# Schaudge/cellranger

Measured on AMD Instinct MI355X. Metric: M reads/sec barcode-correct+UMI-count, higher is better.
Workload: dtype u32/u64 integer keys; f64 posterior

## Files before the change

### cellranger_amd/csrc/common.h

```cpp
#pragma once

#include <hip/hip_runtime.h>

#include <cstdarg>
#include <cstdint>
#include <cstdio>
#include <cstring>
#include <map>
#include <mutex>
#include <set>
#include <string>
#include <vector>

#include "../../include/crgpu.h"

#define CR_WAVE 64
#define CR_SCALAR_N_WITHOUT_FLAGS 40

struct WlTables {
    bool set = false;
    uint32_t n = 0;
    uint32_t bitsA = 0;
    uint32_t bitsB = 0;
    uint32_t *d_offA = nullptr;
// ... 227 lines not shown
        if (_rc != CRGPU_OK) return _rc; \
    } while (0)

#define CR_REQUIRE(ctx, cond, code, ...)                     \
    do {                                                     \
        if (!(cond)) return cr_fail((ctx), (code), __VA_ARGS__); \
    } while (0)

int cr_scratch(crgpu_ctx *ctx, uint64_t bytes, void **out);
void cr_invalidate_range(crgpu_ctx *ctx, const void *p, uint64_t bytes);
void cr_drop_miss_records(crgpu_ctx *ctx);
void cr_drop_miss_records(crgpu_ctx *ctx, MissRecords &r);
bool cr_sweep_plan(uint32_t lo_bit, uint32_t hi_bit, SweepPlan *plan, uint32_t *widths);
uint32_t cr_sort_low_bits(uint32_t total_bits, uint32_t umi_bits);
bool cr_sort_finish_experiment();
int cr_order_runs(crgpu_ctx *ctx, uint64_t *d_keys, uint32_t *d_vals, uint64_t n, uint32_t low_bits, bool *fell_back);
static inline void cr_allow_lds(crgpu_ctx *ctx, const void *kernel, size_t bytes) {
    size_t &have = ctx->lds_attr_done[kernel];
    if (bytes > have) {
        (void)hipFuncSetAttribute(kernel, hipFuncAttributeMaxDynamicSharedMemorySize, (int)bytes);
        have = bytes;
    }
}

int cr_pool_alloc(crgpu_ctx *ctx, void **out, uint64_t bytes);
void cr_pool_free(crgpu_ctx *ctx, void *p);
void cr_pool_release_all(crgpu_ctx *ctx);

hipEvent_t cr_take_event(crgpu_ctx *ctx);
struct CrTimer {
    crgpu_ctx *ctx;
// ... 31 lines not shown
```

### cellranger_amd/csrc/dedup.hip

```cpp
#include "block_utils.h"
#include "common.h"

int cr_scan_small(crgpu_ctx *ctx, uint32_t *d_data, uint64_t n, uint32_t *d_total_out);
int cr_partition_by_owner(crgpu_ctx *ctx, const uint64_t *d_in, uint64_t *d_out, uint64_t n, uint32_t sh_bc,
                          uint32_t n_ranks, const uint32_t *bounds, uint64_t *counts_out);

#define NONE32 0xFFFFFFFFu

struct crgpu_counts {
    uint64_t n_triplets = 0, n_molecules = 0;
    uint32_t *d_bc = nullptr, *d_feature = nullptr, *d_count = nullptr;
    uint64_t *d_mkeys = nullptr;
    uint32_t *d_mreads = nullptr;
    uint32_t *d_corr_reads = nullptr;
    uint32_t *d_filt_reads = nullptr;
    int32_t *d_mprobe = nullptr;
    uint32_t *d_back = nullptr;
    uint32_t n_back = 0;
    uint32_t n_canon = 0;
    KeyLayout layout;
};

extern "C" int crgpu_set_key_layout(crgpu_ctx *ctx, uint32_t n_features, uint32_t umi_len, uint32_t n_libs,
                                    uint32_t multiplexing_lib_mask) {
// ... 604 lines not shown
            const uint64_t i = base + (uint64_t)j * CP_BLOCK + threadIdx.x;
            c += (f[j] && i < hi) ? 1u : 0u;
        }
    }
#pragma unroll
    for (int d = 32; d >= 1; d >>= 1) c += __shfl_xor(c, d);
    if ((threadIdx.x & 63u) == 0) ws[threadIdx.x >> 6] = c;
    __syncthreads();
    if (threadIdx.x == 0) {
        uint32_t t = 0;
        for (int w = 0; w < CP_WAVES; w++) t += ws[w];
        block_counts[blockIdx.x] = t;
    }
}

template <typename Flag, typename Emit>
__global__ __launch_bounds__(CP_BLOCK) void k_cp_write(Flag flag, Emit emit, uint64_t n, uint64_t tile,
                                                       const uint32_t *__restrict__ block_offs) {
    __shared__ uint32_t ws[CP_ITEMS * CP_WAVES];
    __shared__ uint32_t round_total;
    const uint32_t lane = threadIdx.x & 63u, wave = threadIdx.x >> 6;
    const uint64_t lo = (uint64_t)blockIdx.x * tile;
    const uint64_t hi = lo + tile < n ? lo + tile : n;
    uint32_t run = block_offs[blockIdx.x];
    for (uint64_t base = lo; base < hi; base += CP_ROUND) {
        bool f[CP_ITEMS];
        typename Emit::Pre pre[CP_ITEMS];
#pragma unroll
        for (int j = 0; j < CP_ITEMS; j++) {
            const uint64_t i = base + (uint64_t)j * CP_BLOCK + threadIdx.x;
            f[j] = flag(i < hi ? i : hi - 1);
            pre[j] = emit.pre(i < hi ? i : hi - 1);
        }
        uint32_t below[CP_ITEMS];
#pragma unroll
        for (int j = 0; j < CP_ITEMS; j++) {
            const uint64_t i = base + (uint64_t)j * CP_BLOCK + threadIdx.x;
            f[j] = f[j] && i < hi;
            const unsigned long long m = __ballot(f[j]);
// ... 28 lines not shown
    if (nb < 1) nb = 1;
    if (nb > 4096) nb = 4096;
    uint64_t tile = (n + nb - 1) / nb;
    tile = (tile + CP_ROUND - 1) / CP_ROUND * CP_ROUND;
    nb = (n + tile - 1) / tile;
    if (nb < 1) nb = 1;
    *tile_out = tile;
    return (uint32_t)nb;
}

template <typename Flag, typename Emit>
static int compact(crgpu_ctx *ctx, Flag flag, Emit emit, uint64_t n, uint32_t *d_block, uint32_t *d_total_out) {
    uint64_t tile;
    const uint32_t nb = cp_blocks(n, &tile);
    hipLaunchKernelGGL(k_cp_count<Flag>, dim3(nb), dim3(CP_BLOCK), 0, ctx->stream, flag, n, tile, d_block);
    CR_TRY(cr_scan_small(ctx, d_block, nb, d_total_out));
    hipLaunchKernelGGL((k_cp_write<Flag, Emit>), dim3(nb), dim3(CP_BLOCK), 0, ctx->stream, flag, emit, n, tile, d_block);
    CR_HIP(ctx, hipGetLastError());
    return CRGPU_OK;
}

#define ST_CORRECTED 1u
#define ST_LOW 2u
__device__ __forceinline__ uint32_t st_inc1(uint32_t s) { return s >> 2; }
__device__ __forceinline__ void st_or(uint16_t *st, uint64_t k, uint32_t bits) {
    atomicOr(reinterpret_cast<uint32_t *>(st) + (k >> 1), bits << (16u * (uint32_t)(k & 1u)));
}
__device__ __forceinline__ void move_reads(uint32_t *corr, uint16_t *st, uint32_t *inc_all, uint32_t *minidx, uint64_t k,
                                           uint32_t target, uint32_t my_cnt) {
    corr[k] = target;
    st_or(st, k, ST_CORRECTED);
    atomicAdd(reinterpret_cast<uint32_t *>(st) + (target >> 1), 4u << (16u * (target & 1u)));
// ... 142 lines not shown
            c += (head && i < hi) ? 1u : 0u;
        }
    }
#pragma unroll
    for (int d = 32; d >= 1; d >>= 1) c += __shfl_xor(c, d);
    if (lane == 0) ws[wave] = c;
    __syncthreads();
    if (threadIdx.x == 0) {
        uint32_t t = 0;
        for (int w = 0; w < CP_WAVES; w++) t += ws[w];
        block_counts[blockIdx.x] = t;
    }
}

__global__ __launch_bounds__(CP_BLOCK) void k_rl_write(const uint64_t *__restrict__ keys, const uint32_t shift, const uint64_t n,
                                                       const uint64_t tile, const uint32_t *__restrict__ block_offs,
                                                       uint64_t *__restrict__ ukey, uint32_t *__restrict__ upos,
                                                       uint16_t *__restrict__ z_st, uint32_t *__restrict__ z_inc,
                                                       uint32_t *__restrict__ z_min) {
    __shared__ uint32_t ws[CP_ITEMS * CP_WAVES];
    __shared__ uint32_t round_total;
    const uint32_t lane = threadIdx.x & 63u, wave = threadIdx.x >> 6;
    const uint64_t lo = (uint64_t)blockIdx.x * tile;
    const uint64_t hi = lo + tile < n ? lo + tile : n;
    uint32_t run = block_offs[blockIdx.x];
    for (uint64_t base = lo; base < hi; base += CP_ROUND) {
        uint64_t key[CP_ITEMS];
        bool f[CP_ITEMS];
        uint32_t below[CP_ITEMS];
        const uint64_t w0 = base + (uint64_t)wave * (64u * CP_ITEMS);
        const uint64_t wb = w0 > 0 ? (w0 - 1 < n ? w0 - 1 : n - 1) : 0;
        uint64_t carry_key = keys[wb];
        bool carry_valid = w0 > 0;
#pragma unroll
        for (int j = 0; j < CP_ITEMS; j++) {
            const uint64_t i = w0 + (uint64_t)j * 64 + lane;
            key[j] = keys[i < hi ? i : hi - 1];
        }
#pragma unroll
        for (int j = 0; j < CP_ITEMS; j++) {
// ... 10 lines not shown
#pragma unroll
            for (int d = 1; d < CP_ITEMS * CP_WAVES; d <<= 1) {
                const uint32_t y = __shfl_up(x, d);
                if (threadIdx.x >= (uint32_t)d) x += y;
            }
            ws[threadIdx.x] = x - v;
            if (threadIdx.x == CP_ITEMS * CP_WAVES - 1) round_total = x;
        }
        __syncthreads();
#pragma unroll
        for (int j = 0; j < CP_ITEMS; j++)
            if (f[j]) {
                const uint32_t o = run + ws[wave * CP_ITEMS + j] + below[j];
                ukey[o] = key[j];
                upos[o] = (uint32_t)(w0 + (uint64_t)j * 64 + lane);
                if (z_st) {
                    z_st[o] = 0;
                    z_inc[o] = 0u;
                    z_min[o] = 0xFFFFFFFFu;
                }
            }
        run += round_total;
        __syncthreads();
    }
}

static int run_lengths(crgpu_ctx *ctx, const uint64_t *keys, uint32_t shift, uint64_t n, uint64_t *ukey, uint32_t *upos,
                       uint32_t *d_block, uint32_t *d_total_out, uint16_t *z_st = nullptr, uint32_t *z_inc = nullptr,
                       uint32_t *z_min = nullptr) {
    uint64_t tile;
    const uint32_t nb = cp_blocks(n, &tile);
    hipLaunchKernelGGL(k_rl_count, dim3(nb), dim3(CP_BLOCK), 0, ctx->stream, keys, shift, n, tile, d_block);
    CR_TRY(cr_scan_small(ctx, d_block, nb, d_total_out));
    hipLaunchKernelGGL(k_rl_write, dim3(nb), dim3(CP_BLOCK), 0, ctx->stream, keys, shift, n, tile, d_block, ukey, upos, z_st, z_inc,
                       z_min);
    CR_HIP(ctx, hipGetLastError());
    return CRGPU_OK;
}

struct MtCarry {
    uint64_t prefix;
    bool has_mol;
    bool valid;
};

template <typename Flag>
__device__ __forceinline__ MtCarry mt_carry_from_memory(const Flag &flag, const uint64_t *__restrict__ ukey, uint32_t sh_feat,
                                                        uint64_t nd, uint64_t i0) {
    MtCarry c{0ull, false, false};
    if (i0 == 0 || i0 >= nd) return c;
// ... 783 lines not shown
        ~Guard() {
            if (armed) crgpu_counts_free(c, r);
        }
    } guard{ctx, res};

    uint32_t *d_block = ctx->d_sort_hist;
    uint32_t *d_total = ctx->d_scalars + 16;
    if (ctx->dense.valid) {
        res->n_back = ctx->dense.V;
        CR_TRY(cr_pool_alloc(ctx, (void **)&res->d_back, (size_t)ctx->dense.V * sizeof(uint32_t)));
        CR_HIP(ctx, hipMemcpyAsync(res->d_back, ctx->dense.d_back, (size_t)ctx->dense.V * sizeof(uint32_t), hipMemcpyDeviceToDevice,
                                   ctx->stream));
    }

    DevBuf corr_b, incall_b, st_b, minidx_b;
    const bool prezero = ctx->stream2 && n_keys >= (1u << 20) && getenv("CRGPU_PREZERO") != nullptr;
    const bool fused_zero = !prezero && getenv("CRGPU_STATE_FUSED_ZERO") && !getenv("CRGPU_RL_GENERIC") && !cr_sort_finish_experiment();
    const uint64_t st_cap = (prezero || fused_zero) ? n_keys : 0;
    if (fused_zero) {
        CR_TRY(dmalloc(ctx, minidx_b, st_cap * sizeof(uint32_t)));
        CR_TRY(dmalloc(ctx, corr_b, st_cap * sizeof(uint32_t)));
        CR_TRY(dmalloc(ctx, incall_b, st_cap * sizeof(uint32_t)));
        CR_TRY(dmalloc(ctx, st_b, ((st_cap + 1) & ~1ull) * sizeof(uint16_t) + 4));
    }
    if (prezero) {
        CR_TRY(dmalloc(ctx, minidx_b, st_cap * sizeof(uint32_t)));
        CR_TRY(dmalloc(ctx, corr_b, st_cap * sizeof(uint32_t)));
        CR_TRY(dmalloc(ctx, incall_b, st_cap * sizeof(uint32_t)));
        CR_TRY(dmalloc(ctx, st_b, ((st_cap + 1) & ~1ull) * sizeof(uint16_t) + 4));
        CR_HIP(ctx, hipEventRecord(ctx->ev_fork, ctx->stream));
        CR_HIP(ctx, hipStreamWaitEvent(ctx->stream2, ctx->ev_fork, 0));
        CR_HIP(ctx, hipMemsetAsync(incall_b.p, 0, st_cap * sizeof(uint32_t), ctx->stream2));
        CR_HIP(ctx, hipMemsetAsync(st_b.p, 0, ((st_cap + 1) & ~1ull) * sizeof(uint16_t) + 4, ctx->stream2));
        CR_HIP(ctx, hipMemsetAsync(minidx_b.p, 0xFF, st_cap * sizeof(uint32_t), ctx->stream2));
        CR_HIP(ctx, hipEventRecord(ctx->ev_join, ctx->stream2));
    }
    struct PrezeroGuard {
        crgpu_ctx *c;
        bool armed;
        ~PrezeroGuard() {
            if (armed) (void)hipStreamSynchronize(c->stream2);
        }
    } prezero_guard{ctx, prezero};

    DevBuf tmp, vtmp;
    CR_TRY(dmalloc(ctx, tmp, n_keys * sizeof(uint64_t)));
    if (pr.d_vals) CR_TRY(dmalloc(ctx, vtmp, n_keys * sizeof(uint32_t)));
    bool in_tmp = false;
    uint32_t low_left = 0;
    CR_TRY(cr_radix_sort_u64_top(ctx, d_keys_inout, tmp.as<uint64_t>(), pr.d_vals, pr.d_vals ? vtmp.as<uint32_t>() : nullptr, n_keys,
                                 L.total_bits(), &in_tmp, &low_left));
    uint64_t *keys_rw = in_tmp ? tmp.as<uint64_t>() : d_keys_inout;
    uint32_t *vals_rw = pr.d_vals ? (in_tmp ? vtmp.as<uint32_t>() : pr.d_vals) : nullptr;

    DevBuf ukey_b, upos_b;
    CR_TRY(dmalloc(ctx, ukey_b, n_keys * sizeof(uint64_t)));
    CR_TRY(dmalloc(ctx, upos_b, (n_keys + 1) * sizeof(uint32_t)));
    uint64_t *ukey = ukey_b.as<uint64_t>();
    uint32_t *upos = upos_b.as<uint32_t>();
    uint64_t nd = 0;
    bool emitted = false;
    if (low_left) {
        bool fell_back = false;
        if (cr_sort_finish_experiment()) {
            CR_TRY(cr_finish_emit(ctx, keys_rw, vals_rw, n_keys, low_left, ukey, upos, &nd, &fell_back));
            emitted = !fell_back;
        } else {
            CR_TRY(cr_order_runs(ctx, keys_rw, vals_rw, n_keys, low_left, &fell_back));
        }
        if (fell_back) {
            ctx->sort_refinished++;
            uint64_t *other = in_tmp ? d_keys_inout : tmp.as<uint64_t>();
            uint32_t *vother = pr.d_vals ? (in_tmp ? pr.d_vals : vtmp.as<uint32_t>()) : nullptr;
            bool flip = false;
            CR_TRY(cr_radix_sort_u64_full(ctx, keys_rw, other, vals_rw, vother, n_keys, L.total_bits(), &flip));
            if (flip) {
                keys_rw = other;
                vals_rw = vother;
            }
        }
    }
    const uint64_t *keys = keys_rw;
    const uint32_t *vals = vals_rw;
    if (!emitted) {
        uint32_t nd32 = 0;
        {
            CrTimer t(ctx, CRGPU_T_DEDUP, n_keys);
            if (getenv("CRGPU_RL_GENERIC"))
                CR_TRY(compact(ctx, HeadFlag{keys, 1u}, EmitRun{keys, ukey, upos}, n_keys, d_block, d_total));
            else
                CR_TRY(run_lengths(ctx, keys, 1u, n_keys, ukey, upos, d_block, d_total, fused_zero ? st_b.as<uint16_t>() : nullptr,
                                   fused_zero ? incall_b.as<uint32_t>() : nullptr, fused_zero ? minidx_b.as<uint32_t>() : nullptr));
        }
        CR_TRY(read_u32(ctx, d_total, &nd32));
        nd = nd32;
    }

    const uint64_t st_bytes = ((nd + 1) & ~1ull) * sizeof(uint16_t) + 4;
    const bool zeroed = prezero || (fused_zero && !emitted);
    if (!prezero && !fused_zero) {
        CR_TRY(dmalloc(ctx, minidx_b, nd * sizeof(uint32_t)));
        CR_TRY(dmalloc(ctx, corr_b, nd * sizeof(uint32_t)));
        CR_TRY(dmalloc(ctx, incall_b, nd * sizeof(uint32_t)));
        CR_TRY(dmalloc(ctx, st_b, st_bytes));
    } else if (prezero) {
        CR_HIP(ctx, hipStreamWaitEvent(ctx->stream, ctx->ev_join, 0));
        prezero_guard.armed = false;
    }
    uint32_t *corr = corr_b.as<uint32_t>(), *inc_all = incall_b.as<uint32_t>(), *minidx = minidx_b.as<uint32_t>();
    uint16_t *st = st_b.as<uint16_t>();
    const bool overlap = CrFork::enabled(ctx, nd);
    CrFork fork(ctx);
    DevBuf heads_b, giant_b, best_b;
    bool edges_small_on_side = false;
    uint64_t es_tiles = 0;
    uint32_t *es_first = nullptr, *es_last = nullptr, *es_ngiant = nullptr;
    GiantItem *es_items = nullptr;
    if (overlap) {
        CR_HIP(ctx, hipEventRecord(ctx->ev_fork, ctx->stream));
        if (ctx->timing) {
            fork.t0 = cr_take_event(ctx);
            fork.t1 = cr_take_event(ctx);
            CR_HIP(ctx, hipEventRecord(fork.t0, ctx->stream));
        }
    }
    {
        const bool timing_was = ctx->timing;
        if (overlap) ctx->timing = false;
        struct TimingBack {
            crgpu_ctx *c;
            bool v;
            ~TimingBack() { c->timing = v; }
        } timing_back{ctx, timing_was};
        CrTimer t(ctx, CRGPU_T_DEDUP);
        if (!zeroed) {
            CR_HIP(ctx, hipMemsetAsync(inc_all, 0, nd * sizeof(uint32_t), ctx->stream));
            CR_HIP(ctx, hipMemsetAsync(st, 0, st_bytes, ctx->stream));
            CR_HIP(ctx, hipMemsetAsync(minidx, 0xFF, nd * sizeof(uint32_t), ctx->stream));
        }
        const uint64_t n_tiles = (nd + UC_TILE - 1) / UC_TILE;
        CR_TRY(dmalloc(ctx, heads_b, 2 * n_tiles * sizeof(uint32_t)));
        uint32_t *tile_first = heads_b.as<uint32_t>(), *tile_last = tile_first + n_tiles;
#ifndef UC_GRID_WG
#define UC_GRID_WG 5u
#endif
        hipLaunchKernelGGL(k_correct_umis_tiled, dim3(cr_grid(n_tiles, 1, 256u * UC_GRID_WG)), dim3(256), 0, ctx->stream, kl, ukey,
                           upos, nd, n_keys, tile_first, tile_last, corr, st, inc_all, minidx);
        if (n_tiles > 1) {
            const size_t lds_small = (2 * UES_CAP + UES_BUCKETS * 8) * sizeof(uint32_t);
            const size_t lds_large = (2 * UE_CAP + UE_BUCKETS * 8) * sizeof(uint32_t);
            cr_allow_lds(ctx, (const void *)k_correct_umis_edges<false>, lds_large);
            cr_allow_lds(ctx, (const void *)k_giant_probe, lds_large);
            const uint64_t max_items = nd / (UE_CAP / 2) + 16;
            CR_TRY(dmalloc(ctx, giant_b, max_items * sizeof(GiantItem) + 16));
// ... 1091 lines not shown
```

### cellranger_amd/csrc/sort.hip

```cpp
#include <cstdlib>
#include <cstring>
#include <type_traits>
#include <vector>

#include "block_utils.h"
#include <algorithm>

#include "common.h"

#ifdef SORT_NT_IN
#define SORT_LOAD_IN(p) __builtin_nontemporal_load(p)
#else
#define SORT_LOAD_IN(p) (*(p))
#endif
#ifdef SORT_NT_OUT
#define SORT_STORE_OUT(v, p) __builtin_nontemporal_store((v), (p))
#else
#define SORT_STORE_OUT(v, p) (*(p) = (v))
#endif
#ifndef SORT_BLOCK
#define SORT_BLOCK 1024
#endif
#ifndef SORT_ITEMS
#define SORT_ITEMS 16
// ... 936 lines not shown
            if (lane == 0) left = carry;
            const bool has_left = lane > 0 || carry_valid;
            const bool d = i < n && has_left && (key[j] >> low) == (left >> low) && key[j] < left;
            const unsigned long long m = __ballot(d);
            if (lane == 0 && w0 + (uint64_t)j * 64 < n) {
                desc[(w0 >> 6) + j] = m;
                set += m != 0ull;
            }
            carry = __shfl(key[j], 63);
            carry_valid = true;
        }
    }
    if (lane == 0 && set) atomicAdd(n_words_set, set);
}

#define RR_SHORT 12u
template <bool HAS_VALS>
__device__ __forceinline__ void repair_at(uint64_t *__restrict__ keys, uint32_t *__restrict__ vals, uint64_t n, uint32_t low,
                                          const unsigned long long *__restrict__ desc, uint64_t p, uint32_t *__restrict__ bad,
                                          unsigned long long *__restrict__ later_list = nullptr,
                                          uint32_t *__restrict__ later_n = nullptr, uint32_t later_cap = 0u) {
    const uint64_t top = keys[p] >> low;
    uint64_t h = p;
    for (;;) {
        h--;
        if ((desc[h >> 6] >> (h & 63u)) & 1ull) return;
        if (h == 0 || (keys[h - 1] >> low) != top) break;
        if (p - h > OR_MAX) {
            atomicOr(bad, 1u);
            return;
        }
    }
    uint64_t k[RR_SHORT];
    uint32_t v[RR_SHORT];
#pragma unroll
    for (uint32_t j = 0; j < RR_SHORT; j++) {
// ... 2 lines not shown
        v[j] = HAS_VALS ? vals[at] : 0u;
    }
    uint32_t len = RR_SHORT + 1u;
#pragma unroll
    for (uint32_t j = RR_SHORT; j-- > 0;)
        if (h + j >= n || (k[j] >> low) != top) len = j;
    if (len > RR_SHORT) {
        if (h + RR_SHORT < n && (keys[h + RR_SHORT] >> low) == top) {
            if (later_list) {
                const uint32_t slot = atomicAdd(later_n, 1u);
                if (slot < later_cap) {
                    later_list[slot] = h;
                    return;
                }
            }
            or_run_through_memory<HAS_VALS>(keys, vals, n, low, h, bad);
            return;
        }
        len = RR_SHORT;
    }
    uint64_t k0[RR_SHORT];
    uint32_t v0[RR_SHORT];
#pragma unroll
    for (uint32_t j = 0; j < RR_SHORT; j++) {
        k0[j] = k[j];
        v0[j] = v[j];
    }
#pragma unroll
    for (uint32_t t = 0; t < RR_SHORT; t++) {
#pragma unroll
// ... 1 lines not shown
            const bool sw = j + 1 < len && k[j] > k[j + 1];
            const uint64_t a = k[j], b = k[j + 1];
            const uint32_t va = v[j], vb = v[j + 1];
            k[j] = sw ? b : a;
            k[j + 1] = sw ? a : b;
            v[j] = sw ? vb : va;
            v[j + 1] = sw ? va : vb;
        }
    }
#pragma unroll
    for (uint32_t j = 0; j < RR_SHORT; j++)
        if (j < len && (k[j] != k0[j] || (HAS_VALS && v[j] != v0[j]))) {
            keys[h + j] = k[j];
            if (HAS_VALS) vals[h + j] = v[j];
        }
}

#define RR_WORDS 2048u
#define RR_CAP 4096u
template <bool HAS_VALS>
__global__ __launch_bounds__(256) void k_repair_runs(uint64_t *__restrict__ keys, uint32_t *__restrict__ vals, uint64_t n, uint32_t low,
                                                     const unsigned long long *__restrict__ desc, uint64_t n_words,
                                                     uint32_t *__restrict__ bad, unsigned long long *__restrict__ med_list,
                                                     uint32_t *__restrict__ n_med, uint32_t med_cap) {
    __shared__ uint32_t s_n;
    __shared__ uint32_t s_pos[RR_CAP];
    const uint64_t n_tiles = (n_words + RR_WORDS - 1) / RR_WORDS;
    for (uint64_t tile = blockIdx.x; tile < n_tiles; tile += gridDim.x) {
        const uint64_t w0 = tile * RR_WORDS;
        if (threadIdx.x == 0) s_n = 0;
        __syncthreads();
        for (uint32_t j = threadIdx.x; j < RR_WORDS; j += 256) {
            unsigned long long m = w0 + j < n_words ? desc[w0 + j] : 0ull;
            while (m) {
                const uint32_t b = (uint32_t)__ffsll((long long)m) - 1u;
                m &= m - 1ull;
                const uint32_t slot = atomicAdd(&s_n, 1u);
                if (slot < RR_CAP) s_pos[slot] = j * 64u + b;
                else repair_at<HAS_VALS>(keys, vals, n, low, desc, (w0 + j) * 64 + b, bad, med_list, n_med, med_cap);
            }
        }
        __syncthreads();
        const uint32_t cnt = s_n < RR_CAP ? s_n : RR_CAP;
        for (uint32_t t = threadIdx.x; t < cnt; t += 256)
            repair_at<HAS_VALS>(keys, vals, n, low, desc, w0 * 64 + s_pos[t], bad, med_list, n_med, med_cap);
        __syncthreads();
        __syncthreads();
    }
}

template <bool HAS_VALS>
__global__ __launch_bounds__(256) void k_repair_medium_runs(uint64_t *__restrict__ keys, uint32_t *__restrict__ vals, uint64_t n,
                                                            uint32_t low, const unsigned long long *__restrict__ med_list,
                                                            const uint32_t *__restrict__ n_med, uint32_t med_cap,
                                                            unsigned long long *__restrict__ long_list, uint32_t *__restrict__ n_long,
                                                            uint32_t long_cap, uint32_t *__restrict__ bad) {
    const uint32_t lane = threadIdx.x & 63u;
    const uint32_t cnt = *n_med < med_cap ? *n_med : med_cap;
    const uint32_t n_waves = gridDim.x * (blockDim.x >> 6);
    for (uint32_t t = blockIdx.x * (blockDim.x >> 6) + (threadIdx.x >> 6); t < cnt; t += n_waves) {
        const uint64_t h = med_list[t];
        const uint64_t at = h + lane < n ? h + lane : n - 1;
        const uint64_t key = keys[at];
        const uint32_t val = HAS_VALS ? vals[at] : 0u;
        const uint64_t top = __shfl(key, 0) >> low;
        const unsigned long long in = __ballot(h + lane < n && (key >> low) == top);
        const uint32_t len = ~in ? (uint32_t)__ffsll((long long)~in) - 1u : 64u;
        const bool goes_on = len == 64u && h + 64u < n && (keys[h + 64u] >> low) == top;
        if (goes_on) {
            if (lane == 0) {
                const uint32_t slot = long_cap ? atomicAdd(n_long, 1u) : 0xFFFFFFFFu;
                if (slot < long_cap) long_list[slot] = h;
                else or_run_through_memory<HAS_VALS>(keys, vals, n, low, h, bad);
            }
            continue;
        }
        uint32_t rank = 0;
        for (uint32_t i = 0; i < len; i++) {
            const uint64_t ki = __shfl(key, (int)i);
            rank += (ki < key || (ki == key && i < lane)) ? 1u : 0u;
        }
        if (lane < len && rank != lane) {
            keys[h + rank] = key;
            if (HAS_VALS) vals[h + rank] = val;
        }
    }
}

#define RL_CAP 4096u
template <bool HAS_VALS>
__global__ __launch_bounds__(256) void k_repair_long_runs(uint64_t *__restrict__ keys, uint32_t *__restrict__ vals, uint64_t n, uint32_t low,
                                                          const unsigned long long *__restrict__ long_list,
                                                          const uint32_t *__restrict__ n_long, uint32_t long_cap,
                                                          uint32_t *__restrict__ bad) {
    __shared__ uint32_t s_c[RL_CAP];
    __shared__ uint32_t s_v[HAS_VALS ? RL_CAP : 1];
    __shared__ uint32_t s_len;
    const uint32_t tid = threadIdx.x;
    const uint32_t cnt = *n_long < long_cap ? *n_long : long_cap;
    const uint64_t lowmask = (1ull << low) - 1ull;
    for (uint32_t it = blockIdx.x; it < cnt; it += gridDim.x) {
        const uint64_t h = long_list[it];
        const uint64_t top = keys[h] >> low;
        if (tid == 0) s_len = RL_CAP + 1u;
        __syncthreads();
        for (uint32_t j = tid; j <= RL_CAP; j += 256) {
            const bool out = h + j >= n || (keys[h + j] >> low) != top;
            if (out) atomicMin(&s_len, j);
        }
        __syncthreads();
        const uint32_t len = s_len;
        if (len > RL_CAP) {
            if (tid == 0) or_run_through_memory<HAS_VALS>(keys, vals, n, low, h, bad);
            __syncthreads();
            continue;
        }
        uint32_t P = 128;
        while (P < len) P <<= 1;
        for (uint32_t j = tid; j < P; j += 256) {
            s_c[j] = j < len ? ((uint32_t)(keys[h + j] & lowmask) << 12) | j : 0xFFFFFFFFu;
            if (HAS_VALS && j < len) s_v[j] = vals[h + j];
        }
        __syncthreads();
        for (uint32_t k = 2; k <= P; k <<= 1)
            for (uint32_t j = k >> 1; j > 0; j >>= 1) {
                for (uint32_t x = tid; x < P / 2; x += 256) {
                    const uint32_t a = 2u * x - (x & (j - 1u));
                    const uint32_t b = a + j;
                    const bool up = (a & k) == 0u;
                    const uint32_t ca = s_c[a], cb = s_c[b];
                    if ((ca > cb) == up) {
                        s_c[a] = cb;
                        s_c[b] = ca;
                    }
                }
                __syncthreads();
            }
        for (uint32_t j = tid; j < len; j += 256) {
            const uint32_t c = s_c[j];
            if ((c & 4095u) != j) {
                keys[h + j] = (top << low) | (uint64_t)(c >> 12);
                if (HAS_VALS) vals[h + j] = s_v[c & 4095u];
            }
        }
        __syncthreads();
    }
}

int cr_repair_runs(crgpu_ctx *ctx, uint64_t *d_keys, uint32_t *d_vals, uint64_t n, uint32_t low_bits, bool *fell_back) {
    *fell_back = false;
    if (n < 2 || low_bits == 0) return CRGPU_OK;
    uint32_t *d_flag = ctx->d_scalars + 52, *d_set = ctx->d_scalars + 53, *d_nlong = ctx->d_scalars + 54, *d_nmed = ctx->d_scalars + 55;
    const uint64_t n_words = (n + 63) / 64;
    void *d_desc = nullptr, *d_long = nullptr, *d_med = nullptr;
    CR_TRY(cr_pool_alloc(ctx, &d_desc, n_words * sizeof(unsigned long long)));
    struct Rel {
        crgpu_ctx *c;
        void *&p;
        ~Rel() { cr_pool_free(c, p); }
    } rel{ctx, d_desc}, rel_long{ctx, d_long}, rel_med{ctx, d_med};
    uint32_t long_cap = (uint32_t)std::min<uint64_t>(n / 65 + 1, 1u << 20);
    if (cr_pool_alloc(ctx, &d_long, (uint64_t)long_cap * sizeof(unsigned long long)) != CRGPU_OK) {
        d_long = nullptr;
        long_cap = 0;
    }
    uint32_t med_cap = (uint32_t)std::min<uint64_t>(n / 13 + 1, 1u << 24);
    if (cr_pool_alloc(ctx, &d_med, (uint64_t)med_cap * sizeof(unsigned long long)) != CRGPU_OK) {
        d_med = nullptr;
        med_cap = 0;
    }
    {
        CrTimer t(ctx, CRGPU_T_SORT_HIST, n);
        CR_HIP(ctx, hipMemsetAsync(d_flag, 0, 4 * sizeof(uint32_t), ctx->stream));
        const uint64_t n_spans = (n + 64ull * FD_ITEMS - 1) / (64ull * FD_ITEMS);
        hipLaunchKernelGGL(k_find_descents, dim3(cr_grid(n_spans * 64u, 256, 256u * 8u)), dim3(256), 0, ctx->stream, d_keys, n, low_bits,
                           (unsigned long long *)d_desc, d_set);
        const dim3 grid(cr_grid((n_words + RR_WORDS - 1) / RR_WORDS, 1, 256u * 8u));
#define CR_REPAIR_LAUNCH(HV)                                                                                                          \
    hipLaunchKernelGGL(k_repair_runs<HV>, grid, dim3(256), 0, ctx->stream, d_keys, d_vals, n, low_bits,                                   \
                       (const unsigned long long *)d_desc, n_words, d_flag, (unsigned long long *)d_med, d_nmed, med_cap);                \
    if (med_cap)                                                                                                                          \
        hipLaunchKernelGGL(k_repair_medium_runs<HV>, dim3(256u * 8u), dim3(256), 0, ctx->stream, d_keys, d_vals, n, low_bits,             \
                           (const unsigned long long *)d_med, d_nmed, med_cap, (unsigned long long *)d_long, d_nlong, long_cap, d_flag); \
    if (long_cap)                                                                                                                         \
        hipLaunchKernelGGL(k_repair_long_runs<HV>, dim3(256u * 4u), dim3(256), 0, ctx->stream, d_keys, d_vals, n, low_bits,               \
                           (const unsigned long long *)d_long, d_nlong, long_cap, d_flag)
        if (d_vals) {
            CR_REPAIR_LAUNCH(true);
        } else {
            CR_REPAIR_LAUNCH(false);
        }
#undef CR_REPAIR_LAUNCH
        CR_HIP(ctx, hipGetLastError());
    }
    uint32_t flag = 0;
    CR_TRY(crgpu_memcpy_d2h(ctx, &flag, d_flag, sizeof(flag)));
    *fell_back = flag != 0;
    return CRGPU_OK;
}
static int order_low_bits(crgpu_ctx *ctx, uint64_t *d_keys, uint32_t *d_vals, uint64_t n, uint32_t low_bits, bool *fell_back) {
    const char *e = getenv("CRGPU_SORT_FINISH");
    if (e && atoi(e) == 3) return cr_order_runs_r02(ctx, d_keys, d_vals, n, low_bits, fell_back);
    return cr_repair_runs(ctx, d_keys, d_vals, n, low_bits, fell_back);
}
int cr_order_runs(crgpu_ctx *ctx, uint64_t *d_keys, uint32_t *d_vals, uint64_t n, uint32_t low_bits, bool *fell_back) {
    return order_low_bits(ctx, d_keys, d_vals, n, low_bits, fell_back);
}

static int finish_runs(crgpu_ctx *ctx, uint64_t *d_keys, uint32_t *d_vals, uint64_t n, uint32_t low_bits, bool *fell_back) {
    *fell_back = false;
    uint32_t *d_flag = ctx->d_scalars + 52;
    const size_t lds = (size_t)FIN_CAP * 8 + ((FIN_CAP * 2 + 15) & ~15u) + (d_vals ? (size_t)FIN_CAP * 4 : 0);
    {
        CrTimer t(ctx, CRGPU_T_SORT_HIST, n);
        CR_HIP(ctx, hipMemsetAsync(d_flag, 0, sizeof(uint32_t), ctx->stream));
        const dim3 grid(cr_grid((n + FIN_TILE - 1) / FIN_TILE, 1, 256u * 8u));
        if (d_vals) {
            cr_allow_lds(ctx, (const void *)k_finish_runs<true>, lds);
            hipLaunchKernelGGL(k_finish_runs<true>, grid, dim3(256), lds, ctx->stream, d_keys, d_vals, n, low_bits, d_flag);
        } else {
            cr_allow_lds(ctx, (const void *)k_finish_runs<false>, lds);
// ... 396 lines not shown
```

Baseline: 16380.

## Fold run-head counting into descent/repair passes and inline block-offset scan

The descent-finding pass now also counts run heads per compaction block, and the repair kernels apply per-block deltas as they reorder keys. This lets the run-length compaction skip its separate count kernel. The separate small scan launch is also replaced by each write block summing the preceding block counts itself. Finally, the experimental prezero and fused-zero paths are removed. The changes cut kernel launches and a full read of the keys, at the cost of atomics inside repair and a redundant prefix sum in every block.

```diff
diff --git a/cellranger_amd/csrc/common.h b/cellranger_amd/csrc/common.h
--- a/cellranger_amd/csrc/common.h
+++ b/cellranger_amd/csrc/common.h
@@ -265,7 +265,8 @@
 bool cr_sweep_plan(uint32_t lo_bit, uint32_t hi_bit, SweepPlan *plan, uint32_t *widths);
 uint32_t cr_sort_low_bits(uint32_t total_bits, uint32_t umi_bits);
 bool cr_sort_finish_experiment();
-int cr_order_runs(crgpu_ctx *ctx, uint64_t *d_keys, uint32_t *d_vals, uint64_t n, uint32_t low_bits, bool *fell_back);
+int cr_order_runs(crgpu_ctx *ctx, uint64_t *d_keys, uint32_t *d_vals, uint64_t n, uint32_t low_bits, bool *fell_back,
+                  uint32_t *heads = nullptr, uint64_t head_tile = 0, uint32_t head_shift = 0, bool *heads_counted = nullptr);
 static inline void cr_allow_lds(crgpu_ctx *ctx, const void *kernel, size_t bytes) {
     size_t &have = ctx->lds_attr_done[kernel];
     if (bytes > have) {
diff --git a/cellranger_amd/csrc/dedup.hip b/cellranger_amd/csrc/dedup.hip
--- a/cellranger_amd/csrc/dedup.hip
+++ b/cellranger_amd/csrc/dedup.hip
@@ -642,15 +642,39 @@
     }
 }
 
+__device__ __forceinline__ uint32_t cp_block_offset(const uint32_t *__restrict__ counts, uint32_t *__restrict__ total_out) {
+    __shared__ uint32_t s_w[CP_WAVES];
+    const uint32_t b = blockIdx.x;
+    static_assert(CP_BLOCK * 16 >= 4096, "cp_block_offset: one load per thread and slot covers the at most 4096 blocks");
+    uint32_t v[16];
+#pragma unroll
+    for (uint32_t u = 0; u < 16; u++) {
+        const uint32_t i = u * CP_BLOCK + threadIdx.x;
+        v[u] = i < b ? counts[i] : 0u;
+    }
+    uint32_t x = 0;
+#pragma unroll
+    for (uint32_t u = 0; u < 16; u++) x += v[u];
+#pragma unroll
+    for (int d = 32; d >= 1; d >>= 1) x += __shfl_xor(x, d);
+    if ((threadIdx.x & 63u) == 0) s_w[threadIdx.x >> 6] = x;
+    __syncthreads();
+    uint32_t off = 0;
+#pragma unroll
+    for (int w = 0; w < CP_WAVES; w++) off += s_w[w];
+    if (b == gridDim.x - 1 && threadIdx.x == 0 && total_out) *total_out = off + counts[b];
+    return off;
+}
+
 template <typename Flag, typename Emit>
 __global__ __launch_bounds__(CP_BLOCK) void k_cp_write(Flag flag, Emit emit, uint64_t n, uint64_t tile,
-                                                       const uint32_t *__restrict__ block_offs) {
+                                                       const uint32_t *__restrict__ block_counts, uint32_t *__restrict__ total_out) {
     __shared__ uint32_t ws[CP_ITEMS * CP_WAVES];
     __shared__ uint32_t round_total;
     const uint32_t lane = threadIdx.x & 63u, wave = threadIdx.x >> 6;
     const uint64_t lo = (uint64_t)blockIdx.x * tile;
     const uint64_t hi = lo + tile < n ? lo + tile : n;
-    uint32_t run = block_offs[blockIdx.x];
+    uint32_t run = cp_block_offset(block_counts, total_out);
     for (uint64_t base = lo; base < hi; base += CP_ROUND) {
         bool f[CP_ITEMS];
         typename Emit::Pre pre[CP_ITEMS];
@@ -709,8 +733,7 @@
     uint64_t tile;
     const uint32_t nb = cp_blocks(n, &tile);
     hipLaunchKernelGGL(k_cp_count<Flag>, dim3(nb), dim3(CP_BLOCK), 0, ctx->stream, flag, n, tile, d_block);
-    CR_TRY(cr_scan_small(ctx, d_block, nb, d_total_out));
-    hipLaunchKernelGGL((k_cp_write<Flag, Emit>), dim3(nb), dim3(CP_BLOCK), 0, ctx->stream, flag, emit, n, tile, d_block);
+    hipLaunchKernelGGL((k_cp_write<Flag, Emit>), dim3(nb), dim3(CP_BLOCK), 0, ctx->stream, flag, emit, n, tile, d_block, d_total_out);
     CR_HIP(ctx, hipGetLastError());
     return CRGPU_OK;
 }
@@ -883,16 +906,15 @@
 }
 
 __global__ __launch_bounds__(CP_BLOCK) void k_rl_write(const uint64_t *__restrict__ keys, const uint32_t shift, const uint64_t n,
-                                                       const uint64_t tile, const uint32_t *__restrict__ block_offs,
-                                                       uint64_t *__restrict__ ukey, uint32_t *__restrict__ upos,
-                                                       uint16_t *__restrict__ z_st, uint32_t *__restrict__ z_inc,
-                                                       uint32_t *__restrict__ z_min) {
+                                                       const uint64_t tile, const uint32_t *__restrict__ block_counts,
+                                                       uint32_t *__restrict__ total_out, uint64_t *__restrict__ ukey,
+                                                       uint32_t *__restrict__ upos) {
     __shared__ uint32_t ws[CP_ITEMS * CP_WAVES];
     __shared__ uint32_t round_total;
     const uint32_t lane = threadIdx.x & 63u, wave = threadIdx.x >> 6;
     const uint64_t lo = (uint64_t)blockIdx.x * tile;
     const uint64_t hi = lo + tile < n ? lo + tile : n;
-    uint32_t run = block_offs[blockIdx.x];
+    uint32_t run = cp_block_offset(block_counts, total_out);
     for (uint64_t base = lo; base < hi; base += CP_ROUND) {
         uint64_t key[CP_ITEMS];
         bool f[CP_ITEMS];
@@ -933,11 +955,6 @@
                 const uint32_t o = run + ws[wave * CP_ITEMS + j] + below[j];
                 ukey[o] = key[j];
                 upos[o] = (uint32_t)(w0 + (uint64_t)j * 64 + lane);
-                if (z_st) {
-                    z_st[o] = 0;
-                    z_inc[o] = 0u;
-                    z_min[o] = 0xFFFFFFFFu;
-                }
             }
         run += round_total;
         __syncthreads();
@@ -945,14 +962,11 @@
 }
 
 static int run_lengths(crgpu_ctx *ctx, const uint64_t *keys, uint32_t shift, uint64_t n, uint64_t *ukey, uint32_t *upos,
-                       uint32_t *d_block, uint32_t *d_total_out, uint16_t *z_st = nullptr, uint32_t *z_inc = nullptr,
-                       uint32_t *z_min = nullptr) {
+                       uint32_t *d_block, uint32_t *d_total_out, bool counted = false) {
     uint64_t tile;
     const uint32_t nb = cp_blocks(n, &tile);
-    hipLaunchKernelGGL(k_rl_count, dim3(nb), dim3(CP_BLOCK), 0, ctx->stream, keys, shift, n, tile, d_block);
-    CR_TRY(cr_scan_small(ctx, d_block, nb, d_total_out));
-    hipLaunchKernelGGL(k_rl_write, dim3(nb), dim3(CP_BLOCK), 0, ctx->stream, keys, shift, n, tile, d_block, ukey, upos, z_st, z_inc,
-                       z_min);
+    if (!counted) hipLaunchKernelGGL(k_rl_count, dim3(nb), dim3(CP_BLOCK), 0, ctx->stream, keys, shift, n, tile, d_block);
+    hipLaunchKernelGGL(k_rl_write, dim3(nb), dim3(CP_BLOCK), 0, ctx->stream, keys, shift, n, tile, d_block, d_total_out, ukey, upos);
     CR_HIP(ctx, hipGetLastError());
     return CRGPU_OK;
 }
@@ -1766,34 +1780,6 @@
     }
 
     DevBuf corr_b, incall_b, st_b, minidx_b;
-    const bool prezero = ctx->stream2 && n_keys >= (1u << 20) && getenv("CRGPU_PREZERO") != nullptr;
-    const bool fused_zero = !prezero && getenv("CRGPU_STATE_FUSED_ZERO") && !getenv("CRGPU_RL_GENERIC") && !cr_sort_finish_experiment();
-    const uint64_t st_cap = (prezero || fused_zero) ? n_keys : 0;
-    if (fused_zero) {
-        CR_TRY(dmalloc(ctx, minidx_b, st_cap * sizeof(uint32_t)));
-        CR_TRY(dmalloc(ctx, corr_b, st_cap * sizeof(uint32_t)));
-        CR_TRY(dmalloc(ctx, incall_b, st_cap * sizeof(uint32_t)));
-        CR_TRY(dmalloc(ctx, st_b, ((st_cap + 1) & ~1ull) * sizeof(uint16_t) + 4));
-    }
-    if (prezero) {
-        CR_TRY(dmalloc(ctx, minidx_b, st_cap * sizeof(uint32_t)));
-        CR_TRY(dmalloc(ctx, corr_b, st_cap * sizeof(uint32_t)));
-        CR_TRY(dmalloc(ctx, incall_b, st_cap * sizeof(uint32_t)));
-        CR_TRY(dmalloc(ctx, st_b, ((st_cap + 1) & ~1ull) * sizeof(uint16_t) + 4));
-        CR_HIP(ctx, hipEventRecord(ctx->ev_fork, ctx->stream));
-        CR_HIP(ctx, hipStreamWaitEvent(ctx->stream2, ctx->ev_fork, 0));
-        CR_HIP(ctx, hipMemsetAsync(incall_b.p, 0, st_cap * sizeof(uint32_t), ctx->stream2));
-        CR_HIP(ctx, hipMemsetAsync(st_b.p, 0, ((st_cap + 1) & ~1ull) * sizeof(uint16_t) + 4, ctx->stream2));
-        CR_HIP(ctx, hipMemsetAsync(minidx_b.p, 0xFF, st_cap * sizeof(uint32_t), ctx->stream2));
-        CR_HIP(ctx, hipEventRecord(ctx->ev_join, ctx->stream2));
-    }
-    struct PrezeroGuard {
-        crgpu_ctx *c;
-        bool armed;
-        ~PrezeroGuard() {
-            if (armed) (void)hipStreamSynchronize(c->stream2);
-        }
-    } prezero_guard{ctx, prezero};
 
     DevBuf tmp, vtmp;
     CR_TRY(dmalloc(ctx, tmp, n_keys * sizeof(uint64_t)));
@@ -1811,14 +1797,18 @@
     uint64_t *ukey = ukey_b.as<uint64_t>();
     uint32_t *upos = upos_b.as<uint32_t>();
     uint64_t nd = 0;
-    bool emitted = false;
+    bool emitted = false, heads_counted = false;
     if (low_left) {
         bool fell_back = false;
         if (cr_sort_finish_experiment()) {
             CR_TRY(cr_finish_emit(ctx, keys_rw, vals_rw, n_keys, low_left, ukey, upos, &nd, &fell_back));
             emitted = !fell_back;
+        } else if (getenv("CRGPU_RL_GENERIC")) {
+            CR_TRY(cr_order_runs(ctx, keys_rw, vals_rw, n_keys, low_left, &fell_back));
         } else {
-            CR_TRY(cr_order_runs(ctx, keys_rw, vals_rw, n_keys, low_left, &fell_back));
+            uint64_t tile;
+            cp_blocks(n_keys, &tile);
+            CR_TRY(cr_order_runs(ctx, keys_rw, vals_rw, n_keys, low_left, &fell_back, d_block, tile, 1u, &heads_counted));
         }
         if (fell_back) {
             ctx->sort_refinished++;
@@ -1841,24 +1831,17 @@
             if (getenv("CRGPU_RL_GENERIC"))
                 CR_TRY(compact(ctx, HeadFlag{keys, 1u}, EmitRun{keys, ukey, upos}, n_keys, d_block, d_total));
             else
-                CR_TRY(run_lengths(ctx, keys, 1u, n_keys, ukey, upos, d_block, d_total, fused_zero ? st_b.as<uint16_t>() : nullptr,
-                                   fused_zero ? incall_b.as<uint32_t>() : nullptr, fused_zero ? minidx_b.as<uint32_t>() : nullptr));
+                CR_TRY(run_lengths(ctx, keys, 1u, n_keys, ukey, upos, d_block, d_total, heads_counted));
         }
         CR_TRY(read_u32(ctx, d_total, &nd32));
         nd = nd32;
     }
 
     const uint64_t st_bytes = ((nd + 1) & ~1ull) * sizeof(uint16_t) + 4;
-    const bool zeroed = prezero || (fused_zero && !emitted);
-    if (!prezero && !fused_zero) {
-        CR_TRY(dmalloc(ctx, minidx_b, nd * sizeof(uint32_t)));
-        CR_TRY(dmalloc(ctx, corr_b, nd * sizeof(uint32_t)));
-        CR_TRY(dmalloc(ctx, incall_b, nd * sizeof(uint32_t)));
-        CR_TRY(dmalloc(ctx, st_b, st_bytes));
-    } else if (prezero) {
-        CR_HIP(ctx, hipStreamWaitEvent(ctx->stream, ctx->ev_join, 0));
-        prezero_guard.armed = false;
-    }
+    CR_TRY(dmalloc(ctx, minidx_b, nd * sizeof(uint32_t)));
+    CR_TRY(dmalloc(ctx, corr_b, nd * sizeof(uint32_t)));
+    CR_TRY(dmalloc(ctx, incall_b, nd * sizeof(uint32_t)));
+    CR_TRY(dmalloc(ctx, st_b, st_bytes));
     uint32_t *corr = corr_b.as<uint32_t>(), *inc_all = incall_b.as<uint32_t>(), *minidx = minidx_b.as<uint32_t>();
     uint16_t *st = st_b.as<uint16_t>();
     const bool overlap = CrFork::enabled(ctx, nd);
@@ -1885,11 +1868,9 @@
             ~TimingBack() { c->timing = v; }
         } timing_back{ctx, timing_was};
         CrTimer t(ctx, CRGPU_T_DEDUP);
-        if (!zeroed) {
-            CR_HIP(ctx, hipMemsetAsync(inc_all, 0, nd * sizeof(uint32_t), ctx->stream));
-            CR_HIP(ctx, hipMemsetAsync(st, 0, st_bytes, ctx->stream));
-            CR_HIP(ctx, hipMemsetAsync(minidx, 0xFF, nd * sizeof(uint32_t), ctx->stream));
-        }
+        CR_HIP(ctx, hipMemsetAsync(inc_all, 0, nd * sizeof(uint32_t), ctx->stream));
+        CR_HIP(ctx, hipMemsetAsync(st, 0, st_bytes, ctx->stream));
+        CR_HIP(ctx, hipMemsetAsync(minidx, 0xFF, nd * sizeof(uint32_t), ctx->stream));
         const uint64_t n_tiles = (nd + UC_TILE - 1) / UC_TILE;
         CR_TRY(dmalloc(ctx, heads_b, 2 * n_tiles * sizeof(uint32_t)));
         uint32_t *tile_first = heads_b.as<uint32_t>(), *tile_last = tile_first + n_tiles;
diff --git a/cellranger_amd/csrc/sort.hip b/cellranger_amd/csrc/sort.hip
--- a/cellranger_amd/csrc/sort.hip
+++ b/cellranger_amd/csrc/sort.hip
@@ -974,12 +974,70 @@
     if (lane == 0 && set) atomicAdd(n_words_set, set);
 }
 
+static_assert(FD_ITEMS * 256 == 2048, "k_find_descents_heads: a round must be a round of the run-length passes (CP_ROUND)");
+__global__ __launch_bounds__(256) void k_find_descents_heads(const uint64_t *__restrict__ keys, uint64_t n, uint32_t low, uint32_t shift,
+                                                             uint64_t tile, unsigned long long *__restrict__ desc,
+                                                             uint32_t *__restrict__ n_words_set, uint32_t *__restrict__ heads) {
+    __shared__ uint32_t ws[4];
+    const uint32_t lane = threadIdx.x & 63u, wave = threadIdx.x >> 6;
+    const uint64_t lo = (uint64_t)blockIdx.x * tile;
+    const uint64_t hi = lo + tile < n ? lo + tile : n;
+    uint32_t set = 0, c = 0;
+    for (uint64_t base = lo; base < hi; base += 256ull * FD_ITEMS) {
+        const uint64_t w0 = base + (uint64_t)wave * (64u * FD_ITEMS);
+        const uint64_t wb = w0 > 0 ? (w0 - 1 < n ? w0 - 1 : n - 1) : 0;
+        uint64_t key[FD_ITEMS];
+        uint64_t carry = keys[wb];
+        bool carry_valid = w0 > 0;
+#pragma unroll
+        for (int j = 0; j < FD_ITEMS; j++) {
+            const uint64_t i = w0 + (uint64_t)j * 64 + lane;
+            key[j] = keys[i < hi ? i : hi - 1];
+        }
+#pragma unroll
+        for (int j = 0; j < FD_ITEMS; j++) {
+            const uint64_t i = w0 + (uint64_t)j * 64 + lane;
+            uint64_t left = __shfl_up(key[j], 1);
+            if (lane == 0) left = carry;
+            const bool has_left = lane > 0 || carry_valid;
+            const bool d = i < hi && has_left && (key[j] >> low) == (left >> low) && key[j] < left;
+            c += (i < hi && (!has_left || (key[j] >> shift) != (left >> shift))) ? 1u : 0u;
+            const unsigned long long m = __ballot(d);
+            if (lane == 0 && w0 + (uint64_t)j * 64 < hi) {
+                desc[(w0 >> 6) + j] = m;
+                set += m != 0ull;
+            }
+            carry = __shfl(key[j], 63);
+            carry_valid = true;
+        }
+    }
+#pragma unroll
+    for (int d = 32; d >= 1; d >>= 1) c += __shfl_xor(c, d);
+    if (lane == 0) ws[wave] = c;
+    if (lane == 0 && set) atomicAdd(n_words_set, set);
+    __syncthreads();
+    if (threadIdx.x == 0) heads[blockIdx.x] = ws[0] + ws[1] + ws[2] + ws[3];
+}
+
+struct HeadDelta {
+    uint32_t *heads;
+    uint64_t tile;
+    uint32_t shift;
+};
+#define HD_SLOTS 80u
+__device__ __forceinline__ void hd_add(const HeadDelta &hd, int *s_acc, int64_t base, uint64_t pos, int d) {
+    const int64_t b = (int64_t)(pos / hd.tile), s = b - base;
+    if (s >= 0 && s < (int64_t)HD_SLOTS) atomicAdd(&s_acc[s], d);
+    else atomicAdd(&hd.heads[b], (uint32_t)d);
+}
+
 #define RR_SHORT 12u
 template <bool HAS_VALS>
 __device__ __forceinline__ void repair_at(uint64_t *__restrict__ keys, uint32_t *__restrict__ vals, uint64_t n, uint32_t low,
                                           const unsigned long long *__restrict__ desc, uint64_t p, uint32_t *__restrict__ bad,
                                           unsigned long long *__restrict__ later_list = nullptr,
-                                          uint32_t *__restrict__ later_n = nullptr, uint32_t later_cap = 0u) {
+                                          uint32_t *__restrict__ later_n = nullptr, uint32_t later_cap = 0u,
+                                          const HeadDelta hd = HeadDelta{nullptr, 1, 0}, int *s_hd = nullptr, int64_t hd_base = 0) {
     const uint64_t top = keys[p] >> low;
     uint64_t h = p;
     for (;;) {
@@ -1012,6 +1070,7 @@
                     return;
                 }
             }
+            if (hd.heads) atomicOr(bad, 2u);
             or_run_through_memory<HAS_VALS>(keys, vals, n, low, h, bad);
             return;
         }
@@ -1043,6 +1102,13 @@
             keys[h + j] = k[j];
             if (HAS_VALS) vals[h + j] = v[j];
         }
+    if (hd.heads) {
+#pragma unroll
+        for (uint32_t j = 1; j < RR_SHORT; j++) {
+            const bool before = (k0[j] >> hd.shift) != (k0[j - 1] >> hd.shift), after = (k[j] >> hd.shift) != (k[j - 1] >> hd.shift);
+            if (j < len && before != after) hd_add(hd, s_hd, hd_base, h + j, after ? 1 : -1);
+        }
+    }
 }
 
 #define RR_WORDS 2048u
@@ -1051,13 +1117,16 @@
 __global__ __launch_bounds__(256) void k_repair_runs(uint64_t *__restrict__ keys, uint32_t *__restrict__ vals, uint64_t n, uint32_t low,
                                                      const unsigned long long *__restrict__ desc, uint64_t n_words,
                                                      uint32_t *__restrict__ bad, unsigned long long *__restrict__ med_list,
-                                                     uint32_t *__restrict__ n_med, uint32_t med_cap) {
+                                                     uint32_t *__restrict__ n_med, uint32_t med_cap, const HeadDelta hd) {
     __shared__ uint32_t s_n;
     __shared__ uint32_t s_pos[RR_CAP];
+    __shared__ int s_hd[HD_SLOTS];
     const uint64_t n_tiles = (n_words + RR_WORDS - 1) / RR_WORDS;
     for (uint64_t tile = blockIdx.x; tile < n_tiles; tile += gridDim.x) {
         const uint64_t w0 = tile * RR_WORDS;
+        const int64_t hd_base = (int64_t)(w0 * 64 / hd.tile) - 1;
         if (threadIdx.x == 0) s_n = 0;
+        if (threadIdx.x < HD_SLOTS) s_hd[threadIdx.x] = 0;
         __syncthreads();
         for (uint32_t j = threadIdx.x; j < RR_WORDS; j += 256) {
             unsigned long long m = w0 + j < n_words ? desc[w0 + j] : 0ull;
@@ -1066,14 +1135,17 @@
                 m &= m - 1ull;
                 const uint32_t slot = atomicAdd(&s_n, 1u);
                 if (slot < RR_CAP) s_pos[slot] = j * 64u + b;
-                else repair_at<HAS_VALS>(keys, vals, n, low, desc, (w0 + j) * 64 + b, bad, med_list, n_med, med_cap);
+                else repair_at<HAS_VALS>(keys, vals, n, low, desc, (w0 + j) * 64 + b, bad, med_list, n_med, med_cap, hd, s_hd,
+                                         hd_base);
             }
         }
         __syncthreads();
         const uint32_t cnt = s_n < RR_CAP ? s_n : RR_CAP;
         for (uint32_t t = threadIdx.x; t < cnt; t += 256)
-            repair_at<HAS_VALS>(keys, vals, n, low, desc, w0 * 64 + s_pos[t], bad, med_list, n_med, med_cap);
-        __syncthreads();
+            repair_at<HAS_VALS>(keys, vals, n, low, desc, w0 * 64 + s_pos[t], bad, med_list, n_med, med_cap, hd, s_hd, hd_base);
+        __syncthreads();
+        if (hd.heads && threadIdx.x < HD_SLOTS && s_hd[threadIdx.x] != 0)
+            atomicAdd(&hd.heads[hd_base + threadIdx.x], (uint32_t)s_hd[threadIdx.x]);
         __syncthreads();
     }
 }
@@ -1083,7 +1155,7 @@
                                                             uint32_t low, const unsigned long long *__restrict__ med_list,
                                                             const uint32_t *__restrict__ n_med, uint32_t med_cap,
                                                             unsigned long long *__restrict__ long_list, uint32_t *__restrict__ n_long,
-                                                            uint32_t long_cap, uint32_t *__restrict__ bad) {
+                                                            uint32_t long_cap, uint32_t *__restrict__ bad, const HeadDelta hd) {
     const uint32_t lane = threadIdx.x & 63u;
     const uint32_t cnt = *n_med < med_cap ? *n_med : med_cap;
     const uint32_t n_waves = gridDim.x * (blockDim.x >> 6);
@@ -1100,14 +1172,29 @@
             if (lane == 0) {
                 const uint32_t slot = long_cap ? atomicAdd(n_long, 1u) : 0xFFFFFFFFu;
                 if (slot < long_cap) long_list[slot] = h;
-                else or_run_through_memory<HAS_VALS>(keys, vals, n, low, h, bad);
+                else {
+                    if (hd.heads) atomicOr(bad, 2u);
+                    or_run_through_memory<HAS_VALS>(keys, vals, n, low, h, bad);
+                }
             }
             continue;
         }
-        uint32_t rank = 0;
+        uint32_t rank = 0, below = 0;
         for (uint32_t i = 0; i < len; i++) {
             const uint64_t ki = __shfl(key, (int)i);
             rank += (ki < key || (ki == key && i < lane)) ? 1u : 0u;
+            below += (ki >> hd.shift) < (key >> hd.shift) ? 1u : 0u;
+        }
+        if (hd.heads) {
+            const uint64_t left = __shfl_up(key, 1);
+            const bool before = lane > 0 && lane < len && (key >> hd.shift) != (left >> hd.shift);
+            const bool after = lane < len && rank > 0 && below == rank;
+            const uint64_t b0 = h / hd.tile;
+            const unsigned long long a0 = __ballot(after && (h + rank) / hd.tile == b0), a1 = __ballot(after) & ~a0;
+            const unsigned long long e0 = __ballot(before && (h + lane) / hd.tile == b0), e1 = __ballot(before) & ~e0;
+            const int d0 = __popcll(a0) - __popcll(e0), d1 = __popcll(a1) - __popcll(e1);
+            if (lane == 0 && d0) atomicAdd(&hd.heads[b0], (uint32_t)d0);
+            if (lane == 0 && d1) atomicAdd(&hd.heads[b0 + 1], (uint32_t)d1);
         }
         if (lane < len && rank != lane) {
             keys[h + rank] = key;
@@ -1121,10 +1208,11 @@
 __global__ __launch_bounds__(256) void k_repair_long_runs(uint64_t *__restrict__ keys, uint32_t *__restrict__ vals, uint64_t n, uint32_t low,
                                                           const unsigned long long *__restrict__ long_list,
                                                           const uint32_t *__restrict__ n_long, uint32_t long_cap,
-                                                          uint32_t *__restrict__ bad) {
+                                                          uint32_t *__restrict__ bad, const HeadDelta hd) {
     __shared__ uint32_t s_c[RL_CAP];
     __shared__ uint32_t s_v[HAS_VALS ? RL_CAP : 1];
     __shared__ uint32_t s_len;
+    __shared__ int s_hd[4];
     const uint32_t tid = threadIdx.x;
     const uint32_t cnt = *n_long < long_cap ? *n_long : long_cap;
     const uint64_t lowmask = (1ull << low) - 1ull;
@@ -1132,6 +1220,7 @@
         const uint64_t h = long_list[it];
         const uint64_t top = keys[h] >> low;
         if (tid == 0) s_len = RL_CAP + 1u;
+        if (tid < 4) s_hd[tid] = 0;
         __syncthreads();
         for (uint32_t j = tid; j <= RL_CAP; j += 256) {
             const bool out = h + j >= n || (keys[h + j] >> low) != top;
@@ -1140,6 +1229,7 @@
         __syncthreads();
         const uint32_t len = s_len;
         if (len > RL_CAP) {
+            if (tid == 0 && hd.heads) atomicOr(bad, 2u);
             if (tid == 0) or_run_through_memory<HAS_VALS>(keys, vals, n, low, h, bad);
             __syncthreads();
             continue;
@@ -1150,6 +1240,12 @@
             s_c[j] = j < len ? ((uint32_t)(keys[h + j] & lowmask) << 12) | j : 0xFFFFFFFFu;
             if (HAS_VALS && j < len) s_v[j] = vals[h + j];
         }
+        __syncthreads();
+        const uint32_t hs = 12u + hd.shift;
+        const uint64_t b0 = hd.heads ? h / hd.tile : 0;
+        if (hd.heads)
+            for (uint32_t j = tid + 1; j < len; j += 256)
+                if ((s_c[j] >> hs) != (s_c[j - 1] >> hs)) atomicSub(&s_hd[(h + j) / hd.tile - b0], 1);
         __syncthreads();
         for (uint32_t k = 2; k <= P; k <<= 1)
             for (uint32_t j = k >> 1; j > 0; j >>= 1) {
@@ -1171,14 +1267,24 @@
                 keys[h + j] = (top << low) | (uint64_t)(c >> 12);
                 if (HAS_VALS) vals[h + j] = s_v[c & 4095u];
             }
-        }
-        __syncthreads();
-    }
-}
-
-int cr_repair_runs(crgpu_ctx *ctx, uint64_t *d_keys, uint32_t *d_vals, uint64_t n, uint32_t low_bits, bool *fell_back) {
+            if (hd.heads && j > 0 && (c >> hs) != (s_c[j - 1] >> hs)) atomicAdd(&s_hd[(h + j) / hd.tile - b0], 1);
+        }
+        __syncthreads();
+        if (hd.heads && tid < 3 && s_hd[tid] != 0) atomicAdd(&hd.heads[b0 + tid], (uint32_t)s_hd[tid]);
+    }
+}
+
+int cr_repair_runs(crgpu_ctx *ctx, uint64_t *d_keys, uint32_t *d_vals, uint64_t n, uint32_t low_bits, bool *fell_back,
+                   uint32_t *heads = nullptr, uint64_t head_tile = 0, uint32_t head_shift = 0, bool *heads_counted = nullptr) {
     *fell_back = false;
+    if (heads_counted) *heads_counted = false;
     if (n < 2 || low_bits == 0) return CRGPU_OK;
+    if (heads) {
+        CR_REQUIRE(ctx, heads_counted && head_shift >= 1 && head_shift <= low_bits && head_tile % (256u * FD_ITEMS) == 0 &&
+                            head_tile >= RL_CAP / 2 && (n + head_tile - 1) / head_tile <= 4096,
+                   CRGPU_EINVAL, "cr_repair_runs: head counts need 1 <= shift <= low bits and blocks of whole rounds");
+    }
+    const HeadDelta hd{heads, heads ? head_tile : 1, head_shift};
     uint32_t *d_flag = ctx->d_scalars + 52, *d_set = ctx->d_scalars + 53, *d_nlong = ctx->d_scalars + 54, *d_nmed = ctx->d_scalars + 55;
     const uint64_t n_words = (n + 63) / 64;
     void *d_desc = nullptr, *d_long = nullptr, *d_med = nullptr;
@@ -1202,18 +1308,23 @@
         CrTimer t(ctx, CRGPU_T_SORT_HIST, n);
         CR_HIP(ctx, hipMemsetAsync(d_flag, 0, 4 * sizeof(uint32_t), ctx->stream));
         const uint64_t n_spans = (n + 64ull * FD_ITEMS - 1) / (64ull * FD_ITEMS);
-        hipLaunchKernelGGL(k_find_descents, dim3(cr_grid(n_spans * 64u, 256, 256u * 8u)), dim3(256), 0, ctx->stream, d_keys, n, low_bits,
-                           (unsigned long long *)d_desc, d_set);
+        if (heads)
+            hipLaunchKernelGGL(k_find_descents_heads, dim3((uint32_t)((n + head_tile - 1) / head_tile)), dim3(256), 0, ctx->stream, d_keys,
+                               n, low_bits, head_shift, head_tile, (unsigned long long *)d_desc, d_set, heads);
+        else
+            hipLaunchKernelGGL(k_find_descents, dim3(cr_grid(n_spans * 64u, 256, 256u * 8u)), dim3(256), 0, ctx->stream, d_keys, n,
+                               low_bits, (unsigned long long *)d_desc, d_set);
         const dim3 grid(cr_grid((n_words + RR_WORDS - 1) / RR_WORDS, 1, 256u * 8u));
 #define CR_REPAIR_LAUNCH(HV)                                                                                                          \
     hipLaunchKernelGGL(k_repair_runs<HV>, grid, dim3(256), 0, ctx->stream, d_keys, d_vals, n, low_bits,                                   \
-                       (const unsigned long long *)d_desc, n_words, d_flag, (unsigned long long *)d_med, d_nmed, med_cap);                \
+                       (const unsigned long long *)d_desc, n_words, d_flag, (unsigned long long *)d_med, d_nmed, med_cap, hd);            \
     if (med_cap)                                                                                                                          \
         hipLaunchKernelGGL(k_repair_medium_runs<HV>, dim3(256u * 8u), dim3(256), 0, ctx->stream, d_keys, d_vals, n, low_bits,             \
-                           (const unsigned long long *)d_med, d_nmed, med_cap, (unsigned long long *)d_long, d_nlong, long_cap, d_flag); \
+                           (const unsigned long long *)d_med, d_nmed, med_cap, (unsigned long long *)d_long, d_nlong, long_cap, d_flag,  \
+                           hd);                                                                                                           \
     if (long_cap)                                                                                                                         \
         hipLaunchKernelGGL(k_repair_long_runs<HV>, dim3(256u * 4u), dim3(256), 0, ctx->stream, d_keys, d_vals, n, low_bits,               \
-                           (const unsigned long long *)d_long, d_nlong, long_cap, d_flag)
+                           (const unsigned long long *)d_long, d_nlong, long_cap, d_flag, hd)
         if (d_vals) {
             CR_REPAIR_LAUNCH(true);
         } else {
@@ -1224,16 +1335,20 @@
     }
     uint32_t flag = 0;
     CR_TRY(crgpu_memcpy_d2h(ctx, &flag, d_flag, sizeof(flag)));
-    *fell_back = flag != 0;
+    *fell_back = (flag & 1u) != 0;
+    if (heads) *heads_counted = flag == 0;
     return CRGPU_OK;
 }
-static int order_low_bits(crgpu_ctx *ctx, uint64_t *d_keys, uint32_t *d_vals, uint64_t n, uint32_t low_bits, bool *fell_back) {
+static int order_low_bits(crgpu_ctx *ctx, uint64_t *d_keys, uint32_t *d_vals, uint64_t n, uint32_t low_bits, bool *fell_back,
+                          uint32_t *heads = nullptr, uint64_t head_tile = 0, uint32_t head_shift = 0, bool *heads_counted = nullptr) {
+    if (heads_counted) *heads_counted = false;
     const char *e = getenv("CRGPU_SORT_FINISH");
     if (e && atoi(e) == 3) return cr_order_runs_r02(ctx, d_keys, d_vals, n, low_bits, fell_back);
-    return cr_repair_runs(ctx, d_keys, d_vals, n, low_bits, fell_back);
-}
-int cr_order_runs(crgpu_ctx *ctx, uint64_t *d_keys, uint32_t *d_vals, uint64_t n, uint32_t low_bits, bool *fell_back) {
-    return order_low_bits(ctx, d_keys, d_vals, n, low_bits, fell_back);
+    return cr_repair_runs(ctx, d_keys, d_vals, n, low_bits, fell_back, heads, head_tile, head_shift, heads_counted);
+}
+int cr_order_runs(crgpu_ctx *ctx, uint64_t *d_keys, uint32_t *d_vals, uint64_t n, uint32_t low_bits, bool *fell_back, uint32_t *heads,
+                  uint64_t head_tile, uint32_t head_shift, bool *heads_counted) {
+    return order_low_bits(ctx, d_keys, d_vals, n, low_bits, fell_back, heads, head_tile, head_shift, heads_counted);
 }
 
 static int finish_runs(crgpu_ctx *ctx, uint64_t *d_keys, uint32_t *d_vals, uint64_t n, uint32_t low_bits, bool *fell_back) {
```

After: 16610 (median of 6 runs). 1.4% higher.
